# Sir-Teo/MuZero-Go

Measured on AMD Instinct MI355X. Metric: MCTS simulations/sec (whole node) + self-play moves/sec, 9x9 Go, 200 sims/move, higher is better.
Workload: dtype fp32

## Files before the change

### include/mzgo.h

```cpp
#ifndef MZGO_H
#define MZGO_H

#include <stdint.h>

#ifdef __cplusplus
extern "C" {
#endif

enum {
  MZGO_OK = 0,
  MZGO_EINVAL = -1,
  MZGO_EHIP = -2,
  MZGO_ENOWEIGHTS = -3,
  MZGO_EASSERT = -4
};

typedef struct mzgo_config {
  int board_size;
  int latent_dim;
  int num_games;
  int num_simulations;
  int max_moves;
  int compat;
  int temperature_moves;
// ... 36 lines not shown
int mzgo_search(mzgo_engine* eng, const float* root_obs, const double* noise, int G, int move_index,
                int32_t* root_child_visits, double* root_value, void* stream);
int mzgo_reanalyse(mzgo_engine* eng, const int8_t* stones, const uint8_t* invd, const uint8_t* flags,
                   const int32_t* ids, const double* noise, int n, int32_t* visits, double* value,
                   double* policy, void* stream);
int mzgo_tree_export(mzgo_engine* eng, int g, int32_t* n_nodes_host, int32_t* child_host,
                     int32_t* visits_host, double* value_sum_host, float* prior_host,
                     double* root_prior_host, void* stream);

int mzgo_board_reset(mzgo_engine* eng, void* stream);
int mzgo_board_step(mzgo_engine* eng, const int32_t* actions, int32_t* status, double* winner,
                    void* stream);
int mzgo_board_planes(mzgo_engine* eng, double* planes, void* stream);
int mzgo_board_set(mzgo_engine* eng, int g, const int8_t* stones_host, const uint8_t* invd_host,
                   const int32_t* meta_host, void* stream);

int mzgo_selfplay_reset(mzgo_engine* eng, int epoch, void* stream);
int mzgo_selfplay_move(mzgo_engine* eng, void* stream);
int mzgo_selfplay_moves(mzgo_engine* eng, int moves, void* stream);

int mzgo_arena_move(mzgo_engine* eng, mzgo_engine* opponent, void* stream);
int mzgo_arena_moves(mzgo_engine* eng, mzgo_engine* opponent, int moves, void* stream);
int mzgo_selfplay_counters(mzgo_engine* eng, uint64_t* counters_host, void* stream);

int mzgo_selfplay_set_timing(mzgo_engine* eng, int on);
int mzgo_selfplay_launch_times(mzgo_engine* eng, float* boards_ms, float* queue_ms, int cap, int* n_host);
int mzgo_stream_wait_started(mzgo_engine* eng, uint64_t target, void* stream);
int mzgo_tower_timing(mzgo_engine* eng, int enable, double* tower_ms_host, int64_t* towers_host);

int mzgo_dyn_conv_backward_workspace(int B, int C, int64_t* bytes_host);
int mzgo_dyn_conv_backward(const float* grad_out, const float* out, const float* latent, const int64_t* action,
                           const float* emb, const float* weight, int B, int C, int N, float* grad_latent,
                           float* grad_weight, float* grad_bias, void* workspace, int64_t workspace_bytes,
                           void* stream);
int mzgo_conv3x3_relu_forward(const float* x, const int64_t* action, const float* emb, const float* weight,
                              const float* bias, int B, int Cin, int Cout, int N, float* out, void* stream);
int mzgo_conv3x3_backward_workspace(int B, int Cin, int Cout, int64_t* bytes_host);
int mzgo_conv3x3_backward(const float* grad_out, const float* out, const float* x, const int64_t* action,
                          const float* emb, const float* weight, int B, int Cin, int Cout, int N, float* grad_x,
                          float* grad_weight, float* grad_bias, void* workspace, int64_t workspace_bytes,
                          void* stream);
int mzgo_selfplay_inject_noise(mzgo_engine* eng, const double* noise);
int mzgo_selfplay_record_noise(mzgo_engine* eng, double* dst);
int mzgo_tower_record_nodes(mzgo_engine* eng, float* dst);

int mzgo_records_export(mzgo_engine* eng, int g, int32_t* length_host, int32_t* status_host,
// ... 44 lines not shown
```

### muzero-go_amd/csrc/mzgo_capi.hip

```cpp
#include <hip/hip_runtime.h>

#include <algorithm>
#include <cmath>
#include <cstdarg>
#include <cstdio>
#include <cstring>
#include <map>
#include <string>
#include <vector>

#include "../../include/mzgo.h"
#include "mzgo_dispatch.hpp"
#include "mzgo_replay.hpp"
#include "mzgo_tower_host.hpp"

namespace mzgo {
extern const KernelSet kernels_n5_c96, kernels_n6_c96, kernels_n9_c96, kernels_n19_c96, kernels_n6_c128,
    kernels_n6_c64;

size_t conv_bwd_workspace_bytes(int B, int Cin, int Cout);
hipError_t conv_forward(const float* x, const int64_t* action, const float* emb, const float* w, const float* bias,
                        int B, int Cin, int Cout, int N, float* y, hipStream_t s);
hipError_t conv_backward(const float* g, const float* out, const float* x, const int64_t* action, const float* emb,
                         const float* w, int B, int Cin, int Cout, int N, float* gx, float* gw, float* gb,
// ... 160 lines not shown

struct mzgo_engine {
  mzgo_config cfg;
  const KernelSet* ks = nullptr;
  int N = 0, C = 0, A = 0, CELLS = 0, CS = 0, G = 0, S = 0, M = 0;
  int TS = 0;
  std::map<std::string, std::vector<float>> sd;
  std::vector<Spec> spec;
  bool dirty = true;
  float* d_w = nullptr;
  size_t d_w_bytes = 0;
  NetParams np{};
  EngineArrays E{};
  int* d_err = nullptr;
  unsigned* rq_head = nullptr;
  float* d_scr = nullptr;
  size_t scr_floats = 0;
  std::vector<void*> allocs;
  bool timing = false;
  std::vector<hipEvent_t> tev;
  int tn = 0;
  int64_t bytes = 0;
  int epoch = 0;
  const double* noise = nullptr;
  double* noise_out = nullptr;
  TowerHost* tower = nullptr;

  template <class T>
  int alloc(T** p, size_t n) {
    void* v = nullptr;
    hipError_t e = hipMalloc(&v, n * sizeof(T) + 256);
    if (e != hipSuccess) return fail(MZGO_EHIP, "hipMalloc(%zu): %s", n * sizeof(T), hipGetErrorString(e));
    allocs.push_back(v);
    bytes += (int64_t)(n * sizeof(T));
    *p = reinterpret_cast<T*>(v);
    return MZGO_OK;
  }
  ~mzgo_engine() {
    if (tower) {
      for (hipEvent_t ev : tower->evs) (void)hipEventDestroy(ev);
      tower->free_chains();
      for (void* p : {tower->d_wb, (void*)tower->d_wf, (void*)tower->ib, (void*)tower->ob, (void*)tower->s0,
                      (void*)tower->s1, (void*)tower->shp, (void*)tower->sact})
        if (p) (void)hipFree(p);
      if (tower->h_total) (void)hipHostFree(tower->h_total);
      tower->free_batch();
// ... 79 lines not shown
    for (bf16** q : {&t.ib, &t.ob, &t.s0, &t.s1}) {
      HIPCHK(hipMalloc((void**)q, n * sizeof(bf16)));
      HIPCHK(hipMemset(*q, 0, n * sizeof(bf16)));
    }
    HIPCHK(hipMalloc((void**)&t.shp, (size_t)B * t.CC * 3 * t.CS * sizeof(float)));
    HIPCHK(hipMalloc((void**)&t.sact, (size_t)B * sizeof(int)));
    t.scap = B;
    return MZGO_OK;
  }

  SearchParams search_params() const {
    SearchParams sp;
    sp.c_puct = cfg.c_puct; sp.discount = cfg.discount;
    sp.dirichlet_alpha = cfg.dirichlet_alpha; sp.dirichlet_epsilon = cfg.dirichlet_epsilon;
    sp.pass_epsilon = cfg.pass_epsilon; sp.num_simulations = S; sp.compat = cfg.compat;
    sp.variant = cfg.search_variant;
    sp.factored = cfg.direct_dynamics ? 0 : 1;
    sp.seed = cfg.seed;
    sp.helpers = 0;
    sp.net = 0;
    sp.tail = 0;
    const char* lz = getenv("MZGO_LAZY_ROWS");
    sp.lazy_rows = lz && atoi(lz) == 0 ? 0 : 1;
    return sp;
  }
};

void mzgo::replay_engine_view(const mzgo_engine* e, ReplayEngineView* v) {
  const EngineArrays& E = e->E;
  *v = ReplayEngineView{e->N, e->G, e->M, e->C, e->tower ? 1 : 0, e->cfg.game_base, e->epoch,
                        E.stones, E.invd, E.meta, E.rec_stones, E.rec_invd, E.rec_flags, E.rec_action,
                        E.rec_value, E.rec_policy, E.rec_reward, E.final_reward};
}

extern "C" {

const char* mzgo_last_error(void) { return g_err.c_str(); }

void mzgo_default_config(mzgo_config* c, int N) {
  std::memset(c, 0, sizeof *c);
  c->board_size = N;
  c->latent_dim = 96;
  c->num_games = 1;
  c->num_simulations = 128;
  c->max_moves = N * N;
  c->compat = 0;
// ... 99 lines not shown
    chk(e->alloc(&T.in_idx, G));
    chk(e->alloc(&T.out_idx, G));
    chk(e->alloc(&T.root_idx, G));
    chk(e->alloc(&T.act, G));
    chk(e->alloc(&T.job, G * 3));
    chk(e->alloc(&T.simc, G));
    if (rc == MZGO_OK) {
      std::vector<int> ri(G);
      for (size_t g = 0; g < G; ++g) ri[g] = (int)(g * n1);
      if (hipMemcpy(T.root_idx, ri.data(), G * sizeof(int), hipMemcpyHostToDevice) != hipSuccess ||
          hipMemset(T.playing, 0, G * sizeof(int)) != hipSuccess || hipMemset(T.evalact, 0, G * sizeof(int)) != hipSuccess)
        chk(fail(MZGO_EHIP, "tower index setup failed"));
    }
  }
  if (C != 0) {
    chk(e->alloc(&E.prior, TSL * n1 * A));
    chk(e->alloc(&E.child, TSL * n1 * A));
    chk(e->alloc(&E.visits, TSL * n1));
    chk(e->alloc(&E.wsum, TSL * n1));
    chk(e->alloc(&E.root_prior, TSL * A));
    chk(e->alloc(&E.path, TSL * (n1 + 1)));
    chk(e->alloc(&E.nodes, TSL));
    chk(e->alloc(&E.nact, TSL * n1));
    chk(e->alloc(&E.jobs, TSL * job_bytes(A)));
    chk(e->alloc(&E.mpq, 2 * (size_t)G + 1));
    chk(e->alloc(&E.rec_stones, G * M * CELLS));
    chk(e->alloc(&E.rec_invd, G * M * CELLS));
    chk(e->alloc(&E.rec_flags, G * M));
    chk(e->alloc(&E.rec_action, G * M));
    chk(e->alloc(&E.rec_value, G * M));
    chk(e->alloc(&E.rec_policy, G * M * A));
    chk(e->alloc(&E.rec_reward, G * M));
  }
  chk(e->alloc(&E.stones, G * CELLS));
  chk(e->alloc(&E.invd, G * CELLS));
  chk(e->alloc(&E.meta, G * 4));
  chk(e->alloc(&E.game_len, G));
  chk(e->alloc(&E.final_reward, G));
  chk(e->alloc(&E.status, G));
  chk(e->alloc(&E.counters, kCounters));
  chk(e->alloc(&e->d_err, 1));
  chk(e->alloc(&e->rq_head, 1));
#ifdef MZGO_STAMPS
  chk(e->alloc(&E.stamps, TSL * kStampPhases));
  if (E.stamps) (void)hipMemset(E.stamps, 0, TSL * kStampPhases * 8);
#endif
// ... 473 lines not shown

int mzgo_selfplay_counters(mzgo_engine* e, uint64_t* out, void* stream) {
  if (!e || !out) return fail(MZGO_EINVAL, "bad argument");
  hipStream_t s = (hipStream_t)stream;
  unsigned long long c[kCounters] = {};
  std::vector<int> st(e->G);
  HIPCHK(hipMemcpyAsync(c, e->E.counters, sizeof c, hipMemcpyDeviceToHost, s));
  HIPCHK(hipMemcpyAsync(st.data(), e->E.status, e->G * sizeof(int), hipMemcpyDeviceToHost, s));
  HIPCHK(hipStreamSynchronize(s));
  if (int rc = check_chain(e, s)) return rc;
  int playing = 0;
  for (int v : st) playing += v == 0;
  out[0] = c[0]; out[1] = c[1]; out[2] = c[2]; out[3] = (uint64_t)playing; out[4] = c[3]; out[5] = c[4];
  out[6] = c[5]; out[7] = c[6]; out[8] = c[7];
  if (c[8] != 0) {
    const unsigned long long zero = 0;
    HIPCHK(hipMemcpyAsync(e->E.counters + 8, &zero, sizeof zero, hipMemcpyHostToDevice, s));
    HIPCHK(hipStreamSynchronize(s));
    return fail(MZGO_EHIP, "mzgo_stream_wait_started: %llu gate(s) gave up before the target count", c[8]);
  }
  return MZGO_OK;
}

int mzgo_records_export(mzgo_engine* e, int g, int32_t* length, int32_t* status, int8_t* stones,
                        uint8_t* invd, uint8_t* flags, int32_t* action, double* value, double* policy,
                        double* reward, double* final_reward, void* stream) {
  if (!e || e->C == 0 || g < 0 || g >= e->G) return fail(MZGO_EINVAL, "bad argument");
  hipStream_t s = (hipStream_t)stream;
  int meta[4], st = 0;
  HIPCHK(hipMemcpyAsync(meta, e->E.meta + (size_t)g * 4, 16, hipMemcpyDeviceToHost, s));
  HIPCHK(hipMemcpyAsync(&st, e->E.status + g, 4, hipMemcpyDeviceToHost, s));
  HIPCHK(hipStreamSynchronize(s));
  if (int rc = check_chain(e, s)) return rc;
  const int L = meta[3];
  if (length) *length = L;
  if (status) *status = st;
  const size_t M = e->M, CELLS = e->CELLS, A = e->A, base = (size_t)g * M;
  if (L > 0) {
    if (stones) HIPCHK(hipMemcpyAsync(stones, e->E.rec_stones + base * CELLS, L * CELLS, hipMemcpyDeviceToHost, s));
    if (invd) HIPCHK(hipMemcpyAsync(invd, e->E.rec_invd + base * CELLS, L * CELLS, hipMemcpyDeviceToHost, s));
    if (flags) HIPCHK(hipMemcpyAsync(flags, e->E.rec_flags + base, L, hipMemcpyDeviceToHost, s));
    if (action) HIPCHK(hipMemcpyAsync(action, e->E.rec_action + base, L * 4, hipMemcpyDeviceToHost, s));
    if (value) HIPCHK(hipMemcpyAsync(value, e->E.rec_value + base, L * 8, hipMemcpyDeviceToHost, s));
    if (policy) HIPCHK(hipMemcpyAsync(policy, e->E.rec_policy + base * A, L * A * 8, hipMemcpyDeviceToHost, s));
    if (reward) HIPCHK(hipMemcpyAsync(reward, e->E.rec_reward + base, L * 8, hipMemcpyDeviceToHost, s));
  }
// ... 56 lines not shown
```

### muzero-go_amd/csrc/mzgo_common.hpp

```cpp
#pragma once
#include <hip/hip_runtime.h>
#include <stdint.h>

#if !defined(MZGO_DIAG_BUILD) && (defined(MZGO_TCONV_ABL_NODMA) || defined(MZGO_TCONV_ABL_NOBAR))
#error "wrong-result diagnostic switch without -DMZGO_DIAG_BUILD (diagnostic builds: scripts/build_variant.sh)"
#endif

namespace mzgo {


typedef float f32x4 __attribute__((ext_vector_type(4)));
typedef float f32x2 __attribute__((ext_vector_type(2)));

template <int N_, int C_>
struct Geo {
  static constexpr int N = N_;
  static constexpr int C = C_;
  static constexpr int CELLS = N * N;
  static constexpr int A = CELLS + 1;
  static constexpr int CT = (CELLS + 15) / 16;
  static constexpr int CS = CT * 16;
  static constexpr int CPAD = (CS % 32 == 0) ? CS + 16 : CS;
  static constexpr int CINMAX = C > 64 ? C : 64;
  static constexpr int NG = CT >= 3 ? 3 : CT;
// ... 8 lines not shown
  static_assert(C % 16 == 0, "latent_dim must be a multiple of 16");
};

enum : uint32_t { TAG_SELECT = 1, TAG_DIRICHLET = 2, TAG_ACTION = 3, TAG_WEIGHT = 4 };

__host__ __device__ __forceinline__ uint64_t mix64(uint64_t z) {
  z += 0x9E3779B97F4A7C15ull;
  z = (z ^ (z >> 30)) * 0xBF58476D1CE4E5B9ull;
  z = (z ^ (z >> 27)) * 0x94D049BB133111EBull;
  return z ^ (z >> 31);
}
__host__ __device__ __forceinline__ uint64_t stream_key(uint64_t seed, uint32_t game, uint32_t move) {
  return mix64(mix64(seed) ^ ((uint64_t)game << 32 | (uint64_t)move));
}
__host__ __device__ __forceinline__ uint64_t draw(uint64_t key, uint32_t tag, uint64_t idx) {
  return mix64(key ^ ((uint64_t)(tag & 0xFF) << 56) ^ (idx & ((1ull << 56) - 1)));
}
__host__ __device__ __forceinline__ double u01(uint64_t h) { return (double)(h >> 11) * 0x1.0p-53; }
__host__ __device__ __forceinline__ uint32_t randbelow(uint64_t h, uint32_t n) {
  return (uint32_t)(((h >> 32) * (uint64_t)n) >> 32);
}

constexpr int kStampPhases = 96;
constexpr int kStampLds = 91;
#ifdef MZGO_STAMPS
struct Stamp {
  unsigned long long* buf;
  unsigned long long* lds;
  unsigned long long t;
  __device__ explicit Stamp(unsigned long long* b) : buf(b) {
    __shared__ unsigned long long stamp_lds[kStampLds];
    lds = stamp_lds;
    if (threadIdx.x < kStampLds) lds[threadIdx.x] = 0;
    __syncthreads();
    t = __builtin_amdgcn_s_memtime();
  }
  __device__ void lap(int phase) {
    unsigned long long now = __builtin_amdgcn_s_memtime();
    if (threadIdx.x == 0) lds[phase] += now - t;
    t = now;
  }
  unsigned long long xr[kStampPhases - kStampLds] = {};
  __device__ void wave_add(int phase, unsigned long long cycles) {
    if (phase >= kStampLds) {
      if (threadIdx.x == 0) xr[phase - kStampLds] += cycles;
    } else if ((threadIdx.x & 63) == 0) {
      lds[phase] += cycles;
// ... 237 lines not shown
```

### muzero-go_amd/csrc/mzgo_dispatch.hpp

```cpp
#pragma once
#include "mzgo_kernels.hpp"

namespace mzgo {

struct KernelSet {
  int N, C;
  size_t lds_bytes;
  int rep_scratch;
  int shared_batches;
  int tail_convs;
  hipError_t (*initial_inference)(const NetParams&, const float* obs, int B, float* lat, float* val,
                                  float* logits, float* scratch, hipStream_t);
  hipError_t (*recurrent_inference)(const NetParams&, const float* lat, const int64_t* act, int B,
                                    float* nlat, float* rew, float* val, float* logits, int* err,
                                    hipStream_t);
  hipError_t (*search)(const NetParams&, const SearchParams&, const EngineArrays&, const float* obs,
                       const double* noise, int G, int game_base, int move, int* visits,
                       double* value, hipStream_t);
  hipError_t (*board_reset)(const EngineArrays&, int G, hipStream_t);
  hipError_t (*board_step)(const EngineArrays&, int G, const int* act, int* status, double* winner,
                           double komi, hipStream_t);
  hipError_t (*board_planes)(const EngineArrays&, int G, double* planes, hipStream_t);
  hipError_t (*selfplay_move)(const NetParams& np, const NetParams& np_b, const SearchParams&,
                              const PlayParams&, const EngineArrays&, int G, hipStream_t);
  hipError_t (*selfplay_boards)(const SearchParams&, const PlayParams&, const EngineArrays&, int G, hipStream_t);
  hipError_t (*search_queue)(const NetParams& np, const SearchParams&, const PlayParams&, const EngineArrays&,
                             int G, int workgroups, hipStream_t);
  hipError_t (*reanalyse)(const NetParams& np, const SearchParams&, const EngineArrays&, const ReanalyseArgs&,
                          int workgroups, hipStream_t);
  hipError_t (*selfplay_games)(const NetParams& np, const SearchParams&, const PlayParams&, const EngineArrays&,
                               const GamesArgs&, int workgroups, hipStream_t);
};

// ... 41 lines not shown
  }
  static hipError_t boards(const SearchParams& sp, const PlayParams& pp, const EngineArrays& E, int G, hipStream_t s) {
    hipLaunchKernelGGL((k_selfplay_boards<N, C>), dim3(G), dim3(BoardsGeo<Geo<N, C>>::THREADS), 0, s, sp, pp, E);
    return hipGetLastError();
  }
  static hipError_t queue(const NetParams& np, const SearchParams& sp, const PlayParams& pp, const EngineArrays& E,
                          int G, int workgroups, hipStream_t s) {
    hipLaunchKernelGGL((k_search_queue<N, C>), dim3(workgroups), dim3(Geo<N, C>::THREADS), 0, s, np, sp, pp, E, G);
    return hipGetLastError();
  }
  static hipError_t reanalyse(const NetParams& np, const SearchParams& sp, const EngineArrays& E,
                              const ReanalyseArgs& ra, int workgroups, hipStream_t s) {
    hipLaunchKernelGGL((k_reanalyse_queue<N, C>), dim3(workgroups), dim3(Geo<N, C>::THREADS), 0, s, np, sp, E, ra);
    return hipGetLastError();
  }
  static hipError_t games(const NetParams& np, const SearchParams& sp, const PlayParams& pp, const EngineArrays& E,
                          const GamesArgs& ga, int workgroups, hipStream_t s) {
    hipLaunchKernelGGL((k_selfplay_games<N, C>), dim3(workgroups), dim3(Geo<N, C>::THREADS), 0, s, np, sp, pp, E, ga);
    return hipGetLastError();
  }
  static KernelSet table() {
    typedef Geo<N, C> G;
    return KernelSet{N, C, sizeof(Smem<G>), rep_needs_scratch<G>() ? 64 * N * N : 0,
                     Smem<G>::GLOBAL_Y ? 1 : 0, TailConvs<G>::value ? 1 : 0, &ii, &ri, &search, &breset, &bstep,
                     &bplanes,
                     &move, &boards, &queue, &reanalyse, &games};
  }
};

}
```

### muzero-go_amd/csrc/mzgo_kernels.hpp

```cpp
#pragma once
#include "mzgo_jobs.hpp"
#include "mzgo_replay.hpp"

namespace mzgo {

template <class G>
constexpr bool rep_needs_scratch() {
  if constexpr (G::WINO) return Wino<G>::NSTRIP > 1;
  else return false;
}

struct NoRepJobs {
  __device__ bool operator()(int) const { return false; }
};

template <class G, class PlaneFn, class Jobs = NoRepJobs>
__device__ __forceinline__ void representation(Smem<G>& sm, const NetParams& np, PlaneFn planes, float* lat,
                                      int lat_stride, float* scr, unsigned long long* ts = nullptr,
                                      Jobs jobs = Jobs{}) {
  float* mid = rep_needs_scratch<G>() ? scr : lat;
  for (int i = tid_local(); i < 6 * G::CELLS; i += G::THREADS) {
    const int c = i / G::CELLS, j = i - c * G::CELLS;
    sm.u.in[c * G::CPAD + j] = planes(c, j);
  }
// ... 706 lines not shown
    verify_levels<G, Acc>(sm, sp, TV, T, nact, D, I.batch, grp * gs, min(gs, D - grp * gs), I.act, false, st);
  if (mine > 0 && tid_local() < G::AP && vl.failm[tid_local()])
    __hip_atomic_fetch_or(J.h->failm + tid_local(), (unsigned long long)vl.failm[tid_local()], __ATOMIC_RELAXED,
                          __HIP_MEMORY_SCOPE_AGENT);
  return mine;
}
template <class G>
__device__ __forceinline__ int replay_help(Smem<G>& sm, const SearchParams& sp, const EngineArrays& E, int g,
                                           const TreeView& TV, const JobView& J, const JobInfo& I, unsigned bseq) {
  typedef VerifyLds<G, verify_depth<G>()> V;
  V& vl = *reinterpret_cast<V*>(&sm.u.f.wv[0]);
  const double* bvg = J.bv(G::A);
  for (int k = tid_local(); k < I.batch; k += G::THREADS) sm.u.f.bv[k] = bvg[k];
  if (tid_local() < G::AP) vl.failm[tid_local()] = 0;
  __syncthreads();
  const TreeAcc<G, false> T(TV, sm.t);
  return replay_share<G, TreeAcc<G, false>>(sm, sp, TV, T, E.nact + (size_t)g * ((size_t)E.S + 1), J, I, bseq);
}

template <class G, class Acc>
__device__ __forceinline__ int verify_batch(Smem<G>& sm, const SearchParams& sp, const EngineArrays& E, int g,
                                            const TreeView& TV, Acc& T, int* nact, int leaf, int D, int B, int nid,
                                            Stamp* st = nullptr, bool preloaded = false, bool ext = false,
                                            bool* resume = nullptr) {
  if constexpr (!decltype(sm.u.f)::BATCH) {
    return 0;
  } else {
  constexpr int DV = verify_depth<G>();
  typedef VerifyLds<G, DV> V;
  static_assert(sizeof(V) <= sizeof(sm.u.f.wv), "verification arrays overlay the batch buffers");
  V& vl = *reinterpret_cast<V*>(&sm.u.f.wv[0]);
  const int lane = lane_id_local();
  const bool alt = sp.variant == 0;
  const double* bv = sm.u.f.bv;
  if (tid_local() < G::AP) vl.failm[tid_local()] = 0;
  const VerifyPlan vp = verify_plan<G, Acc>(sp, D);
  if (vp.shared) {
    const JobView J = job_of<G>(E, g);
    const JobInfo I = job_info(kJobReplay, vp.ngroups, nid, leaf, vp.gs, sm.t.ract, D, B);
    const unsigned bseq = job_post(J, I, preloaded ? 1u : 0u, [&](unsigned) {
      if (tid_local() < G::AP)
        __hip_atomic_store(J.h->failm + tid_local(), 0ull, __ATOMIC_RELAXED, __HIP_MEMORY_SCOPE_AGENT);
    });
    const int mine = replay_share<G, Acc>(sm, sp, TV, T, nact, J, I, bseq, st, preloaded);
    asm volatile("s_waitcnt vmcnt(0)" ::: "memory");
    __syncthreads();
    job_wait(J, mine, I.units);
// ... 24 lines not shown
      if (d == 0) {
        T.set(0, T.vis(0) + m, vl.wroot[m]);
      } else {
        const int p = T.path(d);
        const bool neg = alt && ((D + 1 - d) & 1);
        double w = T.ws(p);
#pragma unroll 8
        for (int k = 0; k < m; ++k) w = w + (neg ? -bv[k] : bv[k]);
        const int n = T.vis(p) + m;
        T.set(p, n, w);
        if constexpr (Acc::LDS)
          if (d == 1) { sm.t.rvis[sm.t.ract] = n; sm.t.rws[sm.t.ract] = w; }
      }
    }
    wave_lds_sync();
    for (int i = lane; i < m; i += 64) {
      const int ai = sm.u.f.acts[i], n2 = nid + i;
      const double v = 0.0 + bv[i];
      T.set(n2, 1, v);
      nact[n2] = ai;
      T.set_child(leaf, ai, n2);
      if (leaf == 0) T.add_root_child(ai, v);
    }
    if (lane == 0) { sm.t.newest = -1; sm.t.ycache = leaf; }
  }
  __syncthreads();
  if (st) st->lap(74);
  return m;
  }
}

template <class G, class Acc>
__device__ __forceinline__ void sim_loop(Smem<G>& sm, const NetParams& np, const SearchParams& sp,
                                         const EngineArrays& E, int g, const TreeView& TV, uint64_t key) {
  float* pool = pool_of<G>(E, g);
  const size_t node_floats = (size_t)G::C * G::CS;
  float* scratch = pool + (size_t)(E.S + 1) * node_floats;
  int* nact = E.nact + (size_t)g * ((size_t)E.S + 1);
  const int S = sp.num_simulations;
  const bool factored = sp.factored != 0;
  constexpr bool BATCH = decltype(sm.u.f)::BATCH;
  Acc T(TV, sm.t);
  tree_reset_root<G>(T);
  if (tid_local() == 0) {
    sm.t.newest = -1; sm.t.newp_node = -1; sm.t.ycache = -1; sm.t.rowc_node = -1; sm.t.lognode = -1;
  }
  __syncthreads();

  int nodes = 1, convs = 0;
  int rows = 0;
  const bool eager_rows = !(Acc::LDS || shared_jobs<G>(sp) || (decltype(sm.u.f)::GLOBAL_Y && sp.lazy_rows));
  Stamp st(E.stamps);
  int sim = 0;
  if (factored) {
    sim = root_batch<G, Acc>(sm, np, sp, E, g, TV, T, pool, scratch, nact, key, &st);
    if (eager_rows) rows += sim;
    nodes += sim;
    convs += sim > 0 ? 1 : 0;
    st.lap(4);
  }
  bool pending = false;
  int node0 = 0, depth0 = 0;
  while (sim < S) {
    if (!pending) {
      if (wave_id() == 0) {
        const int a = select_leaf<G>(sm.t, T, sp, key, sim, &st, node0, depth0);
        if (lane_id_local() == 0) sm.t.action = a;
        st.wave_add(92, 1);
        st.wave_add(95, (unsigned long long)sm.t.depth);
      }
      __syncthreads();
    }
// ... 84 lines not shown
                                              G::CS, nullptr, &st, G::WINO ? y_lds_target<G>(sm) : nullptr);
        }
        __syncthreads();
        st.lap(82);
        if (!sj && G::WINO && y_lds_target<G>(sm) != nullptr) {
          if (hwready) {
            if (tid_local() < 3 * G::C) sm.u.f.hw[tid_local()] = hwpre;
          } else {
            load_hw<G>(sm, np.head_w);
          }
          if (tid_local() == 0) sm.t.ycache = leaf;
          yc = leaf;
          const int nun1 = sm.t.nunexp;
          if (!(BATCH && (nun1 < S - sim ? nun1 : S - sim) >= 2)) __syncthreads();
        } else {
          yc = -1;
        }
        if (tid_local() == 0) { st.wave_add(59, 1); ++convs; }
      }
      const int nun = sm.t.nunexp;
      const int B = BATCH ? (nun < S - sim ? nun : S - sim) : 1;
      if (BATCH && B >= 2) {
        st.lap(69);
        if (yc != leaf) load_y<G>(sm, yleaf, np.head_w);
        if constexpr (Acc::LDS) {
          if (leaf != 0 && sm.t.rowc_node != leaf) {
            for (int i = tid_local(); i < G::A; i += G::THREADS) {
              sm.t.rowc_child[i] = TV.child[(size_t)leaf * G::A + i];
              sm.t.rowc_prior[i] = TV.prior[(size_t)leaf * G::A + i];
            }
            __syncthreads();
            if (tid_local() == 0) sm.t.rowc_node = leaf;
          }
        }
        if (tid_local() == 0) { sm.u.f.acts[0] = a; sm.t.npick = 1; sm.t.ngrab = 0; }
        __syncthreads();
        st.lap(70);
        uint64_t um[G::AP];
#pragma unroll
        for (int j = 0; j < G::AP; ++j) um[j] = sm.t.umask[j];
#pragma unroll
        for (int j = 0; j < G::AP; ++j)
          if ((a >> 6) == j) um[j] &= ~(1ull << (a & 63));
        if (shared_jobs<G>(sp)) {
          batch_expand_shared<G, Acc::LDS>(sm, np, sp, E, g, TV, B, nid, leaf, sp.net, yleaf, um, nun - 1, 1, key,
                                           sim + 1, &st, prepicked, [&](unsigned) {
                                             if (replay_parallel(true, B, depth))
                                               verify_preload<G, Acc>(sm, sp, TV, T, nact, depth);
                                           });
          st.lap(71);
        } else {
          if (wave_id() == 0) {
            pick_all<G>(um, nun - 1, 1, B - 1, key, sim + 1, sm.u.f.acts, &st);
            wave_lds_sync();
            if (lane_id_local() == 0) __hip_atomic_store(&sm.t.npick, B, __ATOMIC_RELEASE, __HIP_MEMORY_SCOPE_WORKGROUP);
            st.lap(71);
          }
          batch_expand<G, Acc::LDS>(sm, np, sp, TV, B, nid, yleaf, &st);
        }
        __syncthreads();
        st.lap(5);
        if (eager_rows) rows += B;
        if (replay_parallel(shared_jobs<G>(sp), B, depth)) {
          const bool ext = Acc::LDS && B == nun && sim + B < S;
          bool resume = false;
          const int m = verify_batch<G, Acc>(sm, sp, E, g, TV, T, nact, leaf, depth, B, nid, &st, shared_jobs<G>(sp),
                                             ext, &resume);
          if (resume) { node0 = leaf; depth0 = depth; }
          nodes += m;
          sim += m;
          st.lap(63);
          if (tid_local() == 0) { st.wave_add(31, 1); st.wave_add(28, (unsigned long long)m); }
          continue;
        }
        if (wave_id() == 0) {
          const int lane = lane_id_local();
          if (lane == 0) { sm.t.newest = -1; sm.t.ycache = leaf; }
          wave_lds_sync();
          int m = 0;
          const bool alt = sp.variant == 0;
          {
            for (int i = 0; i < B; ++i) {
              const int ai = sm.u.f.acts[i];
              if (i > 0) {
                const int a2 = select_leaf<G>(sm.t, T, sp, key, sim + i, &st);
                st.wave_add(92, 1);
                st.wave_add(95, (unsigned long long)sm.t.depth);
                if (a2 != ai || sm.t.leaf != leaf) {
                  if (lane == 0) sm.t.action = a2;
                  break;
                }
              }
              const int n2 = nid + i;
              if (lane == 0) { T.init(n2); nact[n2] = ai; }
              if (lane == (ai & 63)) T.set_child(leaf, ai, n2);
              if constexpr (!Acc::LDS) asm volatile("s_waitcnt vmcnt(0)" ::: "memory");
              backup<G>(T, depth, n2, sm.u.f.bv[i], alt);
              ++m;
            }
          }
          if (lane == 0) sm.t.bcast = m;
          st.wave_add(93, 1);
          st.wave_add(94, (unsigned long long)m);
        }
        __syncthreads();
        const int m = sm.t.bcast;
        nodes += m;
        sim += m;
        pending = m < B;
        st.lap(63);
        if (tid_local() == 0) { st.wave_add(31, 1); st.wave_add(28, (unsigned long long)m); }
        continue;
      }
      if (tid_local() == 0) {
        T.init(nid);
        sm.t.newest = nid;
        if constexpr (G::TREE_CAP > 0)
          if (nid < G::TREE_CAP) sm.t.rawp[nid >> 5] &= ~(1u << (nid & 31));
      }
      const unsigned long long t_x = st.now();
      expand_heads<G>(sm.u.f, yleaf, yc == leaf, np.etab + (size_t)a * 9 * G::C, np.head_w);
      if (tid_local() == 0) st.wave_add(56, st.now() - t_x);
      ++rows;
      __syncthreads();
      if (tid_local() == 0 && decltype(sm.u.f)::CACHE) sm.t.ycache = leaf;
      heads = sm.u.f.xh;
    } else {
      if (tid_local() == 0) { T.init(nid); sm.t.newest = nid; }
      latent_conv<G, G::C, G::C, 3>(sm, np.w_dyn, np.b_dyn, pool + (size_t)leaf * node_floats, G::CS,
// ... 13 lines not shown
      const unsigned long long t2 = st.now();
      child_priors<G>(sm.t, x, TV.prior + (size_t)nid * G::A, nid, sp.variant);
      st.wave_add(57, t2 - t1);
      st.wave_add(58, st.now() - t2);
    }
    if (wave_id() == 0) {
      float r, v;
      if (factored) heads_value<G, 1>(heads, true, sm.t.hsc, r, v);
      else heads_value<G, Smem<G>::HEAD_PARTS>(heads, true, sm.t.hsc, r, v);
      if (lane_id_local() == (a & 63)) T.set_child(leaf, a, nid);
      if (lane_id_local() == 0) nact[nid] = a;
      backup<G>(T, depth, nid, (double)r + sp.discount * (double)v, sp.variant == 0);
    }
    st.lap(3);
    ++sim;
  }
  __syncthreads();
  st.flush();
  tree_flush<G>(T, nodes);
  if (tid_local() == 0) {
    E.nodes[g] = nodes;
    atomicAdd(&E.counters[3], (unsigned long long)(factored ? convs : nodes - 1));
    atomicAdd(&E.counters[5], (unsigned long long)(factored ? rows : nodes - 1));
  }
  __syncthreads();
}

template <class G, class PlaneFn>
__device__ __forceinline__ void run_search(Smem<G>& sm, const NetParams& np, const SearchParams& sp,
                                  const EngineArrays& E, int g, PlaneFn planes, const double* noise,
                                  uint64_t key, unsigned long long* ts = nullptr, double* noise_out = nullptr) {
  const TreeView TV = TreeViewOf<G>::make(E, g);
  if (tid_local() == 0) sm.t.ngrab = 0;
  build_mask<G>(sm.t, sp.pass_epsilon, [&](int a) { return planes(3, a); });
  float* pool = pool_of<G>(E, g);
  const size_t node_floats = (size_t)G::C * G::CS;
  if (sp.factored && shared_jobs<G>(sp))
    representation<G>(sm, np, planes, pool + (size_t)(E.S + 1) * node_floats, G::CS, pool, ts ? ts + 3 : nullptr,
                      [&](int k) { rep_shared<G>(sm, np, E, g, sp.net, k); return true; });
  else if (sp.factored)
    representation<G>(sm, np, planes, pool + (size_t)(E.S + 1) * node_floats, G::CS, pool, ts ? ts + 3 : nullptr);
  else
    representation<G>(sm, np, planes, pool, G::CS, pool + node_floats, ts ? ts + 3 : nullptr);
#ifdef MZGO_STAMPS
  if (ts) ts[0] = __builtin_amdgcn_s_memtime();
#endif
// ... 482 lines not shown
```

### muzero-go_amd/csrc/mzgo_move.hpp

```cpp
#pragma once
#include "mzgo_board.hpp"
#include "mzgo_search.hpp"

namespace mzgo {

constexpr int kCounters = 9;

struct EngineArrays {
  int S;
  int max_moves;
  float* pool;
  float* prior;
  int* child;
  int* visits;
  double* wsum;
  double* root_prior;
  int* path;
  int* nodes;
  int* nact;
  int8_t* stones;
  uint8_t* invd;
  int* meta;
  int8_t* rec_stones;
  uint8_t* rec_invd;
  uint8_t* rec_flags;
  int* rec_action;
  double* rec_value;
  double* rec_policy;
  double* rec_reward;
  int* game_len;
  double* final_reward;
  int* status;
  unsigned char* jobs;
  int* mpq;
  unsigned long long* counters;
  unsigned long long* stamps;
};

struct PlayParams {
  double temperature;
  int temperature_moves;
  double komi;
// ... 274 lines not shown
```

### muzero-go_amd/csrc/mzgo_search.hpp

```cpp
#pragma once
#include "mzgo_common.hpp"
#include <type_traits>

namespace mzgo {

struct SearchParams {
  double c_puct;
  double discount;
  double dirichlet_alpha;
  double dirichlet_epsilon;
  double pass_epsilon;
  int num_simulations;
  int compat;
  int variant;
  int factored;
  uint64_t seed;
  int helpers;
  int net;
  int tail;
  int lazy_rows;
};

struct TreeView {
  float* prior;
  int* child;
  int* visits;
  double* wsum;
  double* root_prior;
  int* path;
};

constexpr int kRawRow = -2;
constexpr int kLazyRow = -3;
constexpr int kNeedLogits = -4;

template <class G>
struct TreeLds {
  float logits[G::A];
  float fbuf[G::A];
  double dbuf[G::A];
  uint8_t valid[G::A];
  double pass_prior;
  float reward, value;
// ... 6 lines not shown
  int ycache;
  int lognode;
  int lpar, lact;
  float hsc[56];
  int svis[G::TREE_CAP > 0 ? G::TREE_CAP : 1];
  double sws[G::TREE_CAP > 0 ? G::TREE_CAP : 1];
  int spath[G::TREE_CAP > 0 ? G::TREE_CAP : 1];
  int rchild[G::TREE_CAP > 0 ? G::A : 1];
  double rprior[G::TREE_CAP > 0 ? G::A : 1];
  int rvis[G::TREE_CAP > 0 ? G::A : 1];
  double rws[G::TREE_CAP > 0 ? G::A : 1];
  int ract;
  int rowc_node;
  int rowc_child[G::TREE_CAP > 0 ? G::A : 1];
  float rowc_prior[G::TREE_CAP > 0 ? G::A : 1];
  float newp[G::A];
  int newest;
  int newp_node;
  uint32_t rawp[G::TREE_CAP > 0 ? (G::TREE_CAP + 31) / 32 : 1];
  __device__ __forceinline__ bool is_raw(int n) const {
    if constexpr (G::TREE_CAP > 0) return n < G::TREE_CAP && ((rawp[n >> 5] >> (n & 31)) & 1u);
    else return false;
  }
};

template <class G, bool L>
struct TreeAcc {
  static_assert(!L || G::TREE_CAP > 0, "LDS tree needs TREE_CAP");
  static constexpr bool LDS = L;
  TreeView T;
  TreeLds<G>& t;
  __device__ __forceinline__ TreeAcc(const TreeView& tv, TreeLds<G>& tl) : T(tv), t(tl) {}
  __device__ __forceinline__ int vis(int n) const { if constexpr (L) return t.svis[n]; else return T.visits[n]; }
  __device__ __forceinline__ double ws(int n) const { if constexpr (L) return t.sws[n]; else return T.wsum[n]; }
  __device__ __forceinline__ void add(int n, double dv) {
    if constexpr (L) { t.svis[n] += 1; t.sws[n] = t.sws[n] + dv; }
    else { T.visits[n] += 1; T.wsum[n] = T.wsum[n] + dv; }
  }
  __device__ __forceinline__ void init(int n) {
    if constexpr (L) { t.svis[n] = 0; t.sws[n] = 0.0; } else { T.visits[n] = 0; T.wsum[n] = 0.0; }
  }
  __device__ __forceinline__ void set(int n, int vis, double ws) {
    if constexpr (L) { t.svis[n] = vis; t.sws[n] = ws; } else { T.visits[n] = vis; T.wsum[n] = ws; }
  }
  __device__ __forceinline__ int path(int i) const { if constexpr (L) return t.spath[i]; else return T.path[i]; }
  __device__ __forceinline__ void set_path(int i, int n) { if constexpr (L) t.spath[i] = n; else T.path[i] = n; }
// ... 763 lines not shown
  t.depth = depth;
  return -1;
}

template <class G, class Acc>
__device__ __forceinline__ void backup(Acc& T, int depth, int nid, double v, bool alternate = true) {
  const int lane = lane_id_local();
  const int off = nid >= 0 ? 1 : 0;
  const int count = depth + 1 + off;
  const int ract = T.t.ract;
  for (int i = lane; i < count; i += 64) {
    const int node = (off && i == 0) ? nid : T.path(depth - (i - off));
    const double dv = (alternate && (i & 1)) ? -v : v;
    T.add(node, dv);
    if (i == count - 2) T.add_root_child(ract, dv);
  }
  wave_lds_sync();
}

template <class G, class Acc>
__device__ __forceinline__ void tree_reset_root(Acc& T) {
  for (int a = tid_local(); a < G::A; a += G::THREADS) T.set_child(0, a, -1);
  if constexpr (G::TREE_CAP > 0)
    for (int i = tid_local(); i < (G::TREE_CAP + 31) / 32; i += G::THREADS) T.t.rawp[i] = 0u;
  if (tid_local() == 0) { T.init(0); T.set_path(0, 0); }
}

template <class G, class Acc>
__device__ __forceinline__ void tree_flush(Acc& T, int nodes) {
  if constexpr (Acc::LDS) {
    for (int n = tid_local(); n < nodes; n += G::THREADS) {
      T.T.visits[n] = T.t.svis[n];
      T.T.wsum[n] = T.t.sws[n];
    }
  }
}

}
```

### muzero-go_amd/mzgo/_lib.py

```python
import ctypes
import os

import torch

LIB_PATH = os.environ.get("MZGO_LIB") or os.path.join(os.path.dirname(os.path.abspath(__file__)), "libmzgo.so")

MZGO_OK, MZGO_EINVAL, MZGO_EHIP, MZGO_ENOWEIGHTS, MZGO_EASSERT = 0, -1, -2, -3, -4


class Config(ctypes.Structure):

    _fields_ = [
        ("board_size", ctypes.c_int),
        ("latent_dim", ctypes.c_int),
        ("num_games", ctypes.c_int),
        ("num_simulations", ctypes.c_int),
        ("max_moves", ctypes.c_int),
        ("compat", ctypes.c_int),
        ("temperature_moves", ctypes.c_int),
        ("search_variant", ctypes.c_int),
        ("c_puct", ctypes.c_double),
        ("discount", ctypes.c_double),
        ("dirichlet_alpha", ctypes.c_double),
        ("dirichlet_epsilon", ctypes.c_double),
# ... 15 lines not shown
    "mzgo_default_config": (None, [ctypes.POINTER(Config), _I]),
    "mzgo_engine_create": (_I, [ctypes.POINTER(Config), ctypes.POINTER(_P)]),
    "mzgo_engine_destroy": (None, [_P]),
    "mzgo_last_error": (ctypes.c_char_p, []),
    "mzgo_engine_device_bytes": (ctypes.c_int64, [_P]),
    "mzgo_set_weights": (_I, [_P, ctypes.c_char_p, _P, ctypes.POINTER(ctypes.c_int64), _I]),
    "mzgo_weights_ready": (_I, [_P]),
    "mzgo_initial_inference": (_I, [_P, _P, _I, _P, _P, _P, _P]),
    "mzgo_recurrent_inference": (_I, [_P, _P, _P, _I, _P, _P, _P, _P, _P]),
    "mzgo_check_inference_errors": (_I, [_P, _P]),
    "mzgo_search": (_I, [_P, _P, _P, _I, _I, _P, _P, _P]),
    "mzgo_reanalyse": (_I, [_P, _P, _P, _P, _P, _P, _I, _P, _P, _P, _P]),
    "mzgo_tree_export": (_I, [_P, _I, _P, _P, _P, _P, _P, _P, _P]),
    "mzgo_board_reset": (_I, [_P, _P]),
    "mzgo_board_step": (_I, [_P, _P, _P, _P, _P]),
    "mzgo_board_planes": (_I, [_P, _P, _P]),
    "mzgo_board_set": (_I, [_P, _I, _P, _P, _P, _P]),
    "mzgo_selfplay_reset": (_I, [_P, _I, _P]),
    "mzgo_selfplay_move": (_I, [_P, _P]),
    "mzgo_selfplay_moves": (_I, [_P, _I, _P]),
    "mzgo_arena_move": (_I, [_P, _P, _P]),
    "mzgo_arena_moves": (_I, [_P, _P, _I, _P]),
    "mzgo_selfplay_counters": (_I, [_P, _P, _P]),
    "mzgo_selfplay_set_timing": (_I, [_P, _I]),
    "mzgo_selfplay_launch_times": (_I, [_P, _P, _P, _I, _P]),
    "mzgo_stream_wait_started": (_I, [_P, ctypes.c_uint64, _P]),
    "mzgo_tower_timing": (_I, [_P, _I, _P, _P]),
    "mzgo_selfplay_inject_noise": (_I, [_P, _P]),
    "mzgo_selfplay_record_noise": (_I, [_P, _P]),
    "mzgo_tower_record_nodes": (_I, [_P, _P]),
    "mzgo_records_export": (_I, [_P, _I, _P, _P, _P, _P, _P, _P, _P, _P, _P, _P, _P]),
    "mzgo_records_pack": (_I, [_P, _P, ctypes.c_int64, _P, _P]),
    "mzgo_dyn_conv_backward_workspace": (_I, [_I, _I, ctypes.POINTER(ctypes.c_int64)]),
    "mzgo_dyn_conv_backward": (_I, [_P, _P, _P, _P, _P, _P, _I, _I, _I, _P, _P, _P, _P, ctypes.c_int64, _P]),
    "mzgo_conv3x3_relu_forward": (_I, [_P, _P, _P, _P, _P, _I, _I, _I, _I, _P, _P]),
    "mzgo_conv3x3_backward_workspace": (_I, [_I, _I, _I, ctypes.POINTER(ctypes.c_int64)]),
    "mzgo_conv3x3_backward": (_I, [_P, _P, _P, _P, _P, _P, _I, _I, _I, _I, _P, _P, _P, _P, ctypes.c_int64, _P]),
    "mzgo_replay_create": (_I, [_I, _I, _I, _I, ctypes.POINTER(_P)]),
    "mzgo_replay_destroy": (None, [_P]),
    "mzgo_replay_info": (_I, [_P, _P, _P, _P, _P]),
    "mzgo_replay_add_games": (_I, [_P, _P, _P]),
    "mzgo_replay_play_games": (_I, [_P, _P, _I, _I, _P]),
    "mzgo_replay_add": (_I, [_P, _I, _P, _P, _P, _P, _P, _P, _P, ctypes.c_int32, _P]),
    "mzgo_replay_export": (_I, [_P, _I, _P, _P, _P, _P, _P, _P, _P, _P, _P, _P]),
    "mzgo_replay_batch": (_I, [_P, _P, _P, _P, _I, _I, ctypes.c_double, _P, _P, _P, _P, _P, _P, _P, _P, _P]),
    "mzgo_replay_finish_values": (_I, [_P, _P, _P, _P, _I, _P, _P]),
# ... 53 lines not shown
```

### muzero-go_amd/mzgo/engine.py

```python
import ctypes
from dataclasses import dataclass, fields

import numpy as np
import torch

from . import _lib
from ._lib import check, lib, ptr, stream_of


@dataclass
class EngineConfig:

    board_size: int = 9
    latent_dim: int = 96
    num_games: int = 1
    num_simulations: int = 128
    max_moves: int = 0
    compat: str = "reference"
    temperature_moves: int = 15
    search_variant: str = "self_play"
    c_puct: float = 2.5
    discount: float = 0.99
    dirichlet_alpha: float = 0.15
    dirichlet_epsilon: float = 0.02
# ... 200 lines not shown
    def tower_timing(self, enable):
        ms = ctypes.c_double()
        n = ctypes.c_int64()
        check(lib.mzgo_tower_timing(self._h, int(enable), ctypes.byref(ms), ctypes.byref(n)))
        return ms.value, n.value

    def launch_timing(self, enable):
        cap = 4096
        b = np.zeros(cap, np.float32)
        q = np.zeros(cap, np.float32)
        n = ctypes.c_int()
        check(lib.mzgo_selfplay_launch_times(self._h, ptr(b), ptr(q), cap, ctypes.byref(n)))
        check(lib.mzgo_selfplay_set_timing(self._h, int(enable)))
        k = min(n.value, cap)
        return b[:k].tolist(), q[:k].tolist()

    def counters(self):
        out = np.zeros(9, np.uint64)
        check(lib.mzgo_selfplay_counters(self._h, ptr(out), stream_of(self.device)))
        return dict(simulations=int(out[0]), moves=int(out[1]), games_finished=int(out[2]),
                    playing=int(out[3]), dynamics_convs=int(out[4]), tail_convs=int(out[5]),
                    prior_rows=int(out[6]), workgroups_started=int(out[7]), tail_wait_expiries=int(out[8]))

    def wait_started(self, target, stream=None):
        s = stream if stream is not None else torch.cuda.current_stream(self.device)
        check(lib.mzgo_stream_wait_started(self._h, int(target), ctypes.c_void_p(s.cuda_stream)))

    def record(self, g):
        M, CELLS, A = self.M, self.N * self.N, self.A
        length = ctypes.c_int32()
        status = ctypes.c_int32()
        stones = np.empty((M, CELLS), np.int8)
        invd = np.empty((M, CELLS), np.uint8)
        flags = np.empty(M, np.uint8)
        action = np.empty(M, np.int32)
        value = np.empty(M, np.float64)
        policy = np.empty((M, A), np.float64)
        reward = np.empty(M, np.float64)
        final = np.zeros(1, np.float64)
        check(lib.mzgo_records_export(self._h, g, ctypes.byref(length), ctypes.byref(status), ptr(stones),
                                      ptr(invd), ptr(flags), ptr(action), ptr(value), ptr(policy),
                                      ptr(reward), ptr(final), stream_of(self.device)))
        L = length.value
        return dict(length=L, status=status.value, stones=stones[:L], invd=invd[:L], flags=flags[:L],
                    action=action[:L], value=value[:L], policy=policy[:L], reward=reward[:L],
                    final_reward=float(final[0]))
# ... 1 lines not shown
```

Measured before the change: 134.0 million.

## Cache per-leaf batched child values to skip recomputing expansions after cut batches

Adds a per-game global value cache (cval) keyed by leaf and action. When a batched expansion is cut short (m < B), the already computed child values are stored, and an LDS bitmask marks that leaf. A later visit to the same leaf reads those values instead of reloading head weights and recomputing the batch. This costs extra device memory, an LDS bitmask, global writes and reads, and extra counters. It is on by default only for non-tower, non-direct-dynamics configurations with a cache-capable kernel.

```diff
diff --git a/include/mzgo.h b/include/mzgo.h
--- a/include/mzgo.h
+++ b/include/mzgo.h
@@ -82,6 +82,7 @@
 int mzgo_arena_move(mzgo_engine* eng, mzgo_engine* opponent, void* stream);
 int mzgo_arena_moves(mzgo_engine* eng, mzgo_engine* opponent, int moves, void* stream);
 int mzgo_selfplay_counters(mzgo_engine* eng, uint64_t* counters_host, void* stream);
+int mzgo_search_stats(mzgo_engine* eng, uint64_t* stats_host, void* stream);
 
 int mzgo_selfplay_set_timing(mzgo_engine* eng, int on);
 int mzgo_selfplay_launch_times(mzgo_engine* eng, float* boards_ms, float* queue_ms, int cap, int* n_host);
diff --git a/muzero-go_amd/csrc/mzgo_capi.hip b/muzero-go_amd/csrc/mzgo_capi.hip
--- a/muzero-go_amd/csrc/mzgo_capi.hip
+++ b/muzero-go_amd/csrc/mzgo_capi.hip
@@ -206,6 +206,7 @@
   int tn = 0;
   int64_t bytes = 0;
   int epoch = 0;
+  int value_cache = 0;
   const double* noise = nullptr;
   double* noise_out = nullptr;
   TowerHost* tower = nullptr;
@@ -331,6 +332,7 @@
     sp.tail = 0;
     const char* lz = getenv("MZGO_LAZY_ROWS");
     sp.lazy_rows = lz && atoi(lz) == 0 ? 0 : 1;
+    sp.value_cache = value_cache;
     return sp;
   }
 };
@@ -476,6 +478,10 @@
     chk(e->alloc(&E.path, TSL * (n1 + 1)));
     chk(e->alloc(&E.nodes, TSL));
     chk(e->alloc(&E.nact, TSL * n1));
+    const char* vc = getenv("MZGO_VALUE_CACHE");
+    e->value_cache = !TW && !cfg->direct_dynamics && ks->value_cache_cap > 0 && e->S + 2 <= ks->value_cache_cap &&
+                     !(vc && atoi(vc) == 0);
+    if (e->value_cache) chk(e->alloc(&E.cval, TSL * n1 * A));
     chk(e->alloc(&E.jobs, TSL * job_bytes(A)));
     chk(e->alloc(&E.mpq, 2 * (size_t)G + 1));
     chk(e->alloc(&E.rec_stones, G * M * CELLS));
@@ -995,6 +1001,16 @@
   return MZGO_OK;
 }
 
+int mzgo_search_stats(mzgo_engine* e, uint64_t* out, void* stream) {
+  if (!e || !out) return fail(MZGO_EINVAL, "bad argument");
+  hipStream_t s = (hipStream_t)stream;
+  unsigned long long c[3] = {};
+  HIPCHK(hipMemcpyAsync(c, e->E.counters + 9, sizeof c, hipMemcpyDeviceToHost, s));
+  HIPCHK(hipStreamSynchronize(s));
+  out[0] = c[0]; out[1] = c[1]; out[2] = c[2];
+  return MZGO_OK;
+}
+
 int mzgo_records_export(mzgo_engine* e, int g, int32_t* length, int32_t* status, int8_t* stones,
                         uint8_t* invd, uint8_t* flags, int32_t* action, double* value, double* policy,
                         double* reward, double* final_reward, void* stream) {
diff --git a/muzero-go_amd/csrc/mzgo_common.hpp b/muzero-go_amd/csrc/mzgo_common.hpp
--- a/muzero-go_amd/csrc/mzgo_common.hpp
+++ b/muzero-go_amd/csrc/mzgo_common.hpp
@@ -54,7 +54,7 @@
 }
 
 constexpr int kStampPhases = 96;
-constexpr int kStampLds = 91;
+constexpr int kStampLds = 88;
 #ifdef MZGO_STAMPS
 struct Stamp {
   unsigned long long* buf;
diff --git a/muzero-go_amd/csrc/mzgo_dispatch.hpp b/muzero-go_amd/csrc/mzgo_dispatch.hpp
--- a/muzero-go_amd/csrc/mzgo_dispatch.hpp
+++ b/muzero-go_amd/csrc/mzgo_dispatch.hpp
@@ -9,6 +9,7 @@
   int rep_scratch;
   int shared_batches;
   int tail_convs;
+  int value_cache_cap;
   hipError_t (*initial_inference)(const NetParams&, const float* obs, int B, float* lat, float* val,
                                   float* logits, float* scratch, hipStream_t);
   hipError_t (*recurrent_inference)(const NetParams&, const float* lat, const int64_t* act, int B,
@@ -96,7 +97,9 @@
   static KernelSet table() {
     typedef Geo<N, C> G;
     return KernelSet{N, C, sizeof(Smem<G>), rep_needs_scratch<G>() ? 64 * N * N : 0,
-                     Smem<G>::GLOBAL_Y ? 1 : 0, TailConvs<G>::value ? 1 : 0, &ii, &ri, &search, &breset, &bstep,
+                     Smem<G>::GLOBAL_Y ? 1 : 0, TailConvs<G>::value ? 1 : 0,
+                     G::TREE_CAP > 0 && decltype(Smem<G>::u.f)::BATCH && decltype(Smem<G>::u.f)::CACHE ? G::TREE_CAP : 0,
+                     &ii, &ri, &search, &breset, &bstep,
                      &bplanes,
                      &move, &boards, &queue, &reanalyse, &games};
   }
diff --git a/muzero-go_amd/csrc/mzgo_kernels.hpp b/muzero-go_amd/csrc/mzgo_kernels.hpp
--- a/muzero-go_amd/csrc/mzgo_kernels.hpp
+++ b/muzero-go_amd/csrc/mzgo_kernels.hpp
@@ -752,7 +752,7 @@
 __device__ __forceinline__ int verify_batch(Smem<G>& sm, const SearchParams& sp, const EngineArrays& E, int g,
                                             const TreeView& TV, Acc& T, int* nact, int leaf, int D, int B, int nid,
                                             Stamp* st = nullptr, bool preloaded = false, bool ext = false,
-                                            bool* resume = nullptr) {
+                                            bool* resume = nullptr, bool yleaf_lds = true) {
   if constexpr (!decltype(sm.u.f)::BATCH) {
     return 0;
   } else {
@@ -823,7 +823,7 @@
       T.set_child(leaf, ai, n2);
       if (leaf == 0) T.add_root_child(ai, v);
     }
-    if (lane == 0) { sm.t.newest = -1; sm.t.ycache = leaf; }
+    if (lane == 0) { sm.t.newest = -1; if (yleaf_lds) sm.t.ycache = leaf; }
   }
   __syncthreads();
   if (st) st->lap(74);
@@ -849,6 +849,16 @@
   __syncthreads();
 
   int nodes = 1, convs = 0;
+  constexpr bool VCACHE = Acc::LDS && BATCH && decltype(sm.u.f)::CACHE;
+  const bool vcache = VCACHE && factored && sp.value_cache != 0 && E.cval != nullptr && !shared_jobs<G>(sp);
+  int nbcomp = 0, nbcache = 0, ncut = 0;
+  auto cache_cut = [&](int leaf, int m, int B) {
+    double* cv = E.cval + ((size_t)g * ((size_t)E.S + 1) + (size_t)leaf) * G::A;
+    for (int i = m + tid_local() - 64; tid_local() >= 64 && i < B; i += G::THREADS - 64)
+      cv[sm.u.f.acts[i]] = sm.u.f.bv[i];
+    if (tid_local() == 0) sm.t.cvm[leaf >> 5] |= 1u << (leaf & 31);
+    __syncthreads();
+  };
   int rows = 0;
   const bool eager_rows = !(Acc::LDS || shared_jobs<G>(sp) || (decltype(sm.u.f)::GLOBAL_Y && sp.lazy_rows));
   Stamp st(E.stamps);
@@ -979,7 +989,9 @@
       const int B = BATCH ? (nun < S - sim ? nun : S - sim) : 1;
       if (BATCH && B >= 2) {
         st.lap(69);
-        if (yc != leaf) load_y<G>(sm, yleaf, np.head_w);
+        bool cached = false;
+        if constexpr (VCACHE) cached = vcache && sm.t.is_cached(leaf);
+        if (!cached && yc != leaf) load_y<G>(sm, yleaf, np.head_w);
         if constexpr (Acc::LDS) {
           if (leaf != 0 && sm.t.rowc_node != leaf) {
             for (int i = tid_local(); i < G::A; i += G::THREADS) {
@@ -1006,7 +1018,20 @@
                                                verify_preload<G, Acc>(sm, sp, TV, T, nact, depth);
                                            });
           st.lap(71);
+        } else if (cached) {
+          if (wave_id() == 0) {
+            pick_all<G>(um, nun - 1, 1, B - 1, key, sim + 1, sm.u.f.acts, &st);
+            wave_lds_sync();
+            st.lap(71);
+            const double* cv = E.cval + ((size_t)g * ((size_t)E.S + 1) + (size_t)leaf) * G::A;
+            for (int i = lane_id_local(); i < B; i += 64) {
+              sm.u.f.bv[i] = cv[sm.u.f.acts[i]];
+              atomicOr(&sm.t.rawp[(nid + i) >> 5], 1u << ((nid + i) & 31));
+            }
+          }
+          nbcache += B;
         } else {
+          nbcomp += B;
           if (wave_id() == 0) {
             pick_all<G>(um, nun - 1, 1, B - 1, key, sim + 1, sm.u.f.acts, &st);
             wave_lds_sync();
@@ -1022,8 +1047,13 @@
           const bool ext = Acc::LDS && B == nun && sim + B < S;
           bool resume = false;
           const int m = verify_batch<G, Acc>(sm, sp, E, g, TV, T, nact, leaf, depth, B, nid, &st, shared_jobs<G>(sp),
-                                             ext, &resume);
+                                             ext, &resume, !cached);
           if (resume) { node0 = leaf; depth0 = depth; }
+          if constexpr (VCACHE)
+            if (m < B) {
+              if (vcache && !cached && B == nun) cache_cut(leaf, m, B);
+              ++ncut;
+            }
           nodes += m;
           sim += m;
           st.lap(63);
@@ -1032,7 +1062,7 @@
         }
         if (wave_id() == 0) {
           const int lane = lane_id_local();
-          if (lane == 0) { sm.t.newest = -1; sm.t.ycache = leaf; }
+          if (lane == 0) { sm.t.newest = -1; if (!cached) sm.t.ycache = leaf; }
           wave_lds_sync();
           int m = 0;
           const bool alt = sp.variant == 0;
@@ -1062,6 +1092,11 @@
         }
         __syncthreads();
         const int m = sm.t.bcast;
+        if constexpr (VCACHE)
+          if (m < B) {
+            if (vcache && !cached && B == nun) cache_cut(leaf, m, B);
+            ++ncut;
+          }
         nodes += m;
         sim += m;
         pending = m < B;
@@ -1121,6 +1156,9 @@
     E.nodes[g] = nodes;
     atomicAdd(&E.counters[3], (unsigned long long)(factored ? convs : nodes - 1));
     atomicAdd(&E.counters[5], (unsigned long long)(factored ? rows : nodes - 1));
+    if (nbcomp) atomicAdd(&E.counters[9], (unsigned long long)nbcomp);
+    if (nbcache) atomicAdd(&E.counters[10], (unsigned long long)nbcache);
+    if (ncut) atomicAdd(&E.counters[11], (unsigned long long)ncut);
   }
   __syncthreads();
 }
diff --git a/muzero-go_amd/csrc/mzgo_move.hpp b/muzero-go_amd/csrc/mzgo_move.hpp
--- a/muzero-go_amd/csrc/mzgo_move.hpp
+++ b/muzero-go_amd/csrc/mzgo_move.hpp
@@ -4,7 +4,7 @@
 
 namespace mzgo {
 
-constexpr int kCounters = 9;
+constexpr int kCounters = 12;
 
 struct EngineArrays {
   int S;
@@ -18,6 +18,7 @@
   int* path;
   int* nodes;
   int* nact;
+  double* cval;
   int8_t* stones;
   uint8_t* invd;
   int* meta;
diff --git a/muzero-go_amd/csrc/mzgo_search.hpp b/muzero-go_amd/csrc/mzgo_search.hpp
--- a/muzero-go_amd/csrc/mzgo_search.hpp
+++ b/muzero-go_amd/csrc/mzgo_search.hpp
@@ -19,6 +19,7 @@
   int net;
   int tail;
   int lazy_rows;
+  int value_cache;
 };
 
 struct TreeView {
@@ -71,6 +72,11 @@
     if constexpr (G::TREE_CAP > 0) return n < G::TREE_CAP && ((rawp[n >> 5] >> (n & 31)) & 1u);
     else return false;
   }
+  uint32_t cvm[G::TREE_CAP > 0 ? (G::TREE_CAP + 31) / 32 : 1];
+  __device__ __forceinline__ bool is_cached(int n) const {
+    if constexpr (G::TREE_CAP > 0) return n < G::TREE_CAP && ((cvm[n >> 5] >> (n & 31)) & 1u);
+    else return false;
+  }
 };
 
 template <class G, bool L>
@@ -880,7 +886,7 @@
 __device__ __forceinline__ void tree_reset_root(Acc& T) {
   for (int a = tid_local(); a < G::A; a += G::THREADS) T.set_child(0, a, -1);
   if constexpr (G::TREE_CAP > 0)
-    for (int i = tid_local(); i < (G::TREE_CAP + 31) / 32; i += G::THREADS) T.t.rawp[i] = 0u;
+    for (int i = tid_local(); i < (G::TREE_CAP + 31) / 32; i += G::THREADS) { T.t.rawp[i] = 0u; T.t.cvm[i] = 0u; }
   if (tid_local() == 0) { T.init(0); T.set_path(0, 0); }
 }
 
diff --git a/muzero-go_amd/mzgo/_lib.py b/muzero-go_amd/mzgo/_lib.py
--- a/muzero-go_amd/mzgo/_lib.py
+++ b/muzero-go_amd/mzgo/_lib.py
@@ -61,6 +61,7 @@
     "mzgo_arena_move": (_I, [_P, _P, _P]),
     "mzgo_arena_moves": (_I, [_P, _P, _I, _P]),
     "mzgo_selfplay_counters": (_I, [_P, _P, _P]),
+    "mzgo_search_stats": (_I, [_P, _P, _P]),
     "mzgo_selfplay_set_timing": (_I, [_P, _I]),
     "mzgo_selfplay_launch_times": (_I, [_P, _P, _P, _I, _P]),
     "mzgo_stream_wait_started": (_I, [_P, ctypes.c_uint64, _P]),
diff --git a/muzero-go_amd/mzgo/engine.py b/muzero-go_amd/mzgo/engine.py
--- a/muzero-go_amd/mzgo/engine.py
+++ b/muzero-go_amd/mzgo/engine.py
@@ -246,6 +246,11 @@
                     playing=int(out[3]), dynamics_convs=int(out[4]), tail_convs=int(out[5]),
                     prior_rows=int(out[6]), workgroups_started=int(out[7]), tail_wait_expiries=int(out[8]))
 
+    def search_stats(self):
+        out = np.zeros(3, np.uint64)
+        check(lib.mzgo_search_stats(self._h, ptr(out), stream_of(self.device)))
+        return dict(batch_children_computed=int(out[0]), batch_children_cached=int(out[1]), batches_cut=int(out[2]))
+
     def wait_started(self, target, stream=None):
         s = stream if stream is not None else torch.cuda.current_stream(self.device)
         check(lib.mzgo_stream_wait_started(self._h, int(target), ctypes.c_void_p(s.cuda_stream)))
```

Measured after the change: 137.6 million (median of 6 runs). 1.03x the previous value.
